# os-hxfan/BayesNN_FPGA

Measured on AMD Instinct MI355X. Metric: MCD-samples/sec (T x images/s) + ECE, ResNet-18 multi-exit T=100, higher is better.
Workload: dtype f16; 1 GPU; ResNet18MCEarlyExit C=10 dropout=block+exit p=0.25, batch 250 x T=100 (BASELINE configs[2]); batch=250, T=100, chunk_samples=102, batches_in_flight=2, hipgraph=False, macro_batches=1, pipe=2 eager batches in flight (the probed step is over 1.5 ms)

## Files before the change

### bayesnn_fpga_amd/csrc/conv3x3_s2.hip

```cpp
#include <cstdlib>

#include "conv_epilogue.h"
#include "kernels.h"

typedef _Float16 half8 __attribute__((ext_vector_type(8)));

#ifndef S2_DIRECT
#define S2_DIRECT 1
#endif
#ifndef S2_RELAX0
#define S2_RELAX0 0
#endif
#ifndef S2_DRAIN_STORES
#define S2_DRAIN_STORES 0
#endif
#ifndef S2_WSPLIT
#define S2_WSPLIT 0
#endif
#ifndef S2_STORE_SC1
#define S2_STORE_SC1 0
#endif
#ifndef S2_PIECE_PHASE
#define S2_PIECE_PHASE 1
#endif
// ... 90 lines not shown
        return (s == 0 || s == 4) ? 1 : ((s == 5 && !last) ? 1 : 0);
    }
    __host__ __device__ static constexpr int p_issued(int s, bool last) { return ((s <= 4 || !last) ? pieces_at(s) : 0) + bits_at(s, last); }
    __host__ __device__ static constexpr int wait_n(int S, bool last) {
        int n = 0;
        for (int j = S - (NST - 2); j <= S; ++j) {
            const bool prev = j < 0;
            const int sj = prev ? j + 9 : j;
            const bool lastj = last && !prev;
            if (j > S - (NST - 2)) n += w_issued(sj, lastj) ? WPI : 0;
            n += p_issued(sj, lastj);
        }
        return n;
    }
    static constexpr int WST = CT * 64;
    static constexpr int PIECE = 512 * 16;
    static constexpr int P_OFF = (NST - 1) * WST;
    static constexpr int E_OFF = P_OFF + PRO * PIECE;
    static constexpr int E_BYTES = 65536;
    static constexpr int END_PIECES = P_OFF + NPT * PIECE;
    static constexpr int WL_OFF = (END_PIECES + WST > E_OFF + E_BYTES ? END_PIECES : E_OFF + E_BYTES - WST);
    static constexpr int BN_OFF = WL_OFF + WST;
    static constexpr int BITS_OFF = BN_OFF + 2 * BN_MAX * 4 + 128;
    __host__ __device__ static constexpr int first_due(int S) {
        for (int k = 0; k < NPT; ++k)
            if (pstep(k) + 3 == S || pstep(k) + 3 == S + 9) return k;
        return -1;
    }
    static constexpr int NSLOT = MSK ? (S2_BITS_GROUP ? 3 : 6) : 0;
    __host__ __device__ static constexpr int slot(int k) { return S2_BITS_GROUP ? grp(k) : (k >= PRO ? k - PRO : (k < NA ? (k < 2 ? k : 5) : 2 + (k - NA))); }
    static_assert(!MSK || (NA == 3 && NB == 2 && NOWN == 5 && NPT == 10), "keep-bit slot plan");
    static constexpr int LUT_OFF = BITS_OFF + NSLOT * 2048;
    static constexpr int LDS_BYTES = LUT_OFF + (MSK && S2_MASK_LUT ? 4096 : 0);
    static_assert(BN_OFF - E_OFF >= E_BYTES, "epilogue staging area");
    static_assert(LDS_BYTES <= 160 * 1024, "LDS");
    __host__ __device__ static constexpr int wstage_off(int st) { return st == NST - 1 ? WL_OFF : st * WST; }
    __host__ __device__ static constexpr int p_img(int p) { return p / (TW * TW); }
    __host__ __device__ static constexpr int p_ox(int p) { return 4 * ((p >> 4) % (TW / 4)) + (p & 3); }
    __host__ __device__ static constexpr int p_oy(int p) { return 4 * (((p >> 4) / (TW / 4)) % (TW / 4)) + ((p >> 2) & 3); }
    static constexpr int BR = TW / 4, BI = BR * BR;
    __host__ __device__ static constexpr int cell_delta(int pl, int j) {
        return (j / BI) * rows(pl) * cols(pl) + 4 * ((j % BI) / BR) * cols(pl) + 4 * ((j % BI) % BR);
    }
};

__host__ __device__ constexpr int s2_plane(int s) { return s < 4 ? 0 : (s < 6 ? 1 : (s < 8 ? 2 : 3)); }
__host__ __device__ constexpr int s2_dy(int s) { return (s == 2 || s == 3 || s == 5) ? 1 : 0; }
__host__ __device__ constexpr int s2_dx(int s) { return (s == 1 || s == 3 || s == 7) ? 1 : 0; }
__host__ __device__ constexpr int s2_tap(int s) {
    constexpr int t[9] = {0, 2, 6, 8, 1, 7, 3, 5, 4};
    return t[s];
}

template <int TW, bool BF, bool IMAP, bool MSK = false, int CT_ = 256>
__global__ __launch_bounds__(512, 1) void conv3x3_s2_kernel(ConvArgs a, int n_tiles) {
    using G = S2Geom<TW, (TW == 4 ? 3 : S2_NST_BIG), MSK, CT_>;
    static_assert(!MSK || (TW == 16 && !IMAP), "masked input: one image per tile, the ordinary form");
    constexpr int CT = G::CT, IMGS = G::IMGS, NPT = G::NPT, PRO = G::PRO, NST = G::NST;
    constexpr bool HALF = CT == 128;
    constexpr int TI = 4, TP = HALF ? 4 : 8, JB = TP / 2;
    typedef float accv __attribute__((ext_vector_type(4)));
    __shared__ __attribute__((aligned(16))) char smem[G::LDS_BYTES];
    char* const pbuf = smem + G::P_OFF;
    float* const bn_scale = (float*)(smem + G::BN_OFF);
    float* const bn_bias = bn_scale + G::BN_MAX;

    const int tid = threadIdx.x;
    const int lane = tid & 63;
    const int wave = __builtin_amdgcn_readfirstlane(tid >> 6);
    const int l16 = lane & 15, kq = lane >> 4;
    const int g = wave >> 2, wc = (wave >> 1) & 1, wp = wave & 1;

    const int n_ctiles = a.Cout / CT;
    const int n_ptiles = (a.N + IMGS - 1) / IMGS;
    const int Ktot = 9 * a.Cin;
    const int nC = a.Cin / 32;
    const int split = a.wgt_b ? a.split : a.Cout;

    for (int c = tid; c < a.Cout; c += 512) {
        const bool second = c >= split;
        const float* sp = second ? a.scale_b : a.scale;
        const float* bp = second ? a.bias_b : a.bias;
        const int cc = second ? c - split : c;
        bn_scale[c] = (sp ? sp[cc] : 1.f) * a.out_mul;
        bn_bias[c] = bp ? bp[cc] : 0.f;
    }
    if constexpr (MSK && S2_MASK_LUT) {
        if (tid < 256) {
            typedef unsigned int u32x4_l __attribute__((ext_vector_type(4)));
            u32x4_l m;
#pragma unroll
            for (int i = 0; i < 4; ++i) m[i] = (((tid >> (2 * i)) & 1) ? 0xffffu : 0u) | (((tid >> (2 * i + 1)) & 1) ? 0xffff0000u : 0u);
            *(u32x4_l*)(smem + G::LUT_OFF + tid * 16) = m;
        }
    }
    __syncthreads();

    const int a_off = ((HALF ? 0 : g * 128) + wc * 64 + (S2_DIRECT ? 8 * (l16 >> 2) + (l16 & 3) : l16)) * 64 + ((kq ^ (((l16 >> 2) & 1) << 1)) << 4);
#define A_TILE(I) (S2_DIRECT ? (32 * ((I) >> 1) + 4 * ((I) & 1)) * 64 : (I) * 16 * 64)
    const int by = l16 >> 2, bx = l16 & 3;
    const int pbase = HALF ? (g * 2 + wp) * 64 : wp * 128;
    int boff[4];
#pragma unroll
    for (int pl = 0; pl < 4; ++pl) {
        const int wave_cell = G::cell0(pl) + (G::p_img(pbase) * G::rows(pl) + G::p_oy(pbase)) * G::cols(pl) + G::p_ox(pbase);
        boff[pl] = G::P_OFF + (wave_cell + by * G::cols(pl) + bx) * 64 + ((kq ^ ((by & 1) << 1)) << 4);
    }

    const unsigned HWC = (unsigned)a.H * a.W * a.Cin;
    constexpr unsigned OOB = 0xfffffff0u;
    unsigned pre[NPT];
#pragma unroll
    for (int k = 0; k < NPT; ++k) {
        const int q = tid + 512 * k;
        const int cell = q >> 2, pos = q & 3;
        const int pl = G::lo(k) == G::hi(k) ? G::lo(k) : (cell < G::cell0(G::hi(k)) ? G::lo(k) : G::hi(k));
        const int pyl = pl < 2 ? 1 : 0, pxl = (pl == 0 || pl == 2) ? 1 : 0;
        const int RQ = (TW + pyl) * (TW + pxl), Q = TW + pxl;
        const int lc = cell - (pl == 0 ? 0 : (pl == 1 ? G::cell0(1) : (pl == 2 ? G::cell0(2) : G::cell0(3))));
        const int img = lc / RQ, rm = lc - img * RQ;
        const int y = rm / Q, x = rm - y * Q;
        const int iy = 2 * y - pyl, ix = 2 * x - pxl;
        const bool ok = lc < IMGS * RQ && (unsigned)iy < (unsigned)a.H && (unsigned)ix < (unsigned)a.W;
        const unsigned inoff = (MSK && a.lazy_planar) ? (unsigned)((iy * a.W + (ix & 1) * (a.W >> 1) + (ix >> 1)) * 32 + ((pos ^ ((y & 1) << 1)) << 3))
                                                      : (unsigned)((iy * a.W + ix) * a.Cin + ((pos ^ ((y & 1) << 1)) << 3));
        pre[k] = !ok ? OOB : (IMAP ? ((unsigned)img << 24) | inoff : 2u * ((unsigned)img * HWC + inoff));
    }
    int* const row_tabs = (int*)(smem + G::BN_OFF + 2 * G::BN_MAX * 4);
    int tsel = 0;
    const unsigned woff = 2u * ((unsigned)(tid >> 2) * Ktot + (((tid & 3) ^ (((tid >> (S2_DIRECT ? 5 : 4)) & 1) << 1)) << 3));
    const unsigned wbytes = 2u * 128u * Ktot;
    const unsigned cmul = (MSK && a.lazy_planar) ? (unsigned)(a.H * a.W) : 1u;
    __amdgpu_buffer_rsrc_t rs_w0, rs_w1, rs_in, rs_bits;

    int ch0 = 0, n0 = 0;

#define BLDS16(RSRC, VOFF, SOFF, LDSPTR) \
    __builtin_amdgcn_raw_ptr_buffer_load_lds((RSRC), (__attribute__((address_space(3))) void*)(LDSPTR), 16, (VOFF), (SOFF), 0, 0)
#define ISSUE_W_HALF(KOFF, ST, I)                                                                            \
    {                                                                                                        \
        const unsigned so_ = __builtin_amdgcn_readfirstlane(2u * (unsigned)(KOFF));                          \
        if ((I) == 0) BLDS16(rs_w0, woff, so_, smem + G::wstage_off(ST) + (0 * 512 + wave * 64) * 16);       \
        else BLDS16(rs_w1, woff, so_, smem + G::wstage_off(ST) + (1 * 512 + wave * 64) * 16);                \
    }
#define ISSUE_W(KOFF, ST)                                                                                    \
    {                                                                                                        \
        ISSUE_W_HALF(KOFF, ST, 0);                                                                           \
        if (!HALF) ISSUE_W_HALF(KOFF, ST, 1);                                                                \
    }
#define ISSUE_P(K, C0)                                                                                       \
    {                                                                                                        \
        unsigned o_ = pre[K];                                                                                \
        if constexpr (IMAP) {                                                                                \
            const int row_ = row_tabs[tsel * 16 + ((pre[K] >> 24) & 15)];                                    \
            o_ = (pre[K] == OOB || row_ < 0) ? OOB : 2u * ((unsigned)row_ * HWC + (pre[K] & 0xffffffu));     \
        }                                                                                                    \
        if (!S2_ABL_NOPATCH) BLDS16(rs_in, o_, __builtin_amdgcn_readfirstlane(2u * (unsigned)(C0) * cmul), pbuf + ((K) * 512 + wave * 64) * 16); \
        if constexpr (MSK && !S2_ABL_NOBITS && !S2_BITS_GROUP) {                                             \
             \
             \
             \
            unsigned bo_ = pre[K];                                                                           \
            asm volatile("" : "+v"(bo_));                                                                    \
            __builtin_amdgcn_raw_ptr_buffer_load_lds(rs_bits, (__attribute__((address_space(3))) void*)(smem + G::BITS_OFF + G::slot(K) * 2048 + wave * 256), \
                                                     4, (bo_ >> 4) & ~3u, __builtin_amdgcn_readfirstlane(((unsigned)(C0) * cmul) >> 3), 0, 0); \
        }                                                                                                    \
    }
#define ISSUE_BITS(GRP, PA, PB, PC, PD, CB, ADD0)                                                            \
    if constexpr (MSK && !S2_ABL_NOBITS && S2_BITS_GROUP) {                                                  \
        int p4_ = tid & 3;                                                                                   \
        asm volatile("" : "+v"(p4_));                                                                        \
        unsigned bo_ = p4_ == 0 ? pre[PA] : (p4_ == 1 ? pre[PB] : ((PC) >= 0 ? (p4_ == 2 ? pre[(PC) < 0 ? 0 : (PC)] : pre[(PD) < 0 ? 0 : (PD)]) : OOB)); \
        bo_ = ((bo_ >> 4) & ~3u) + (p4_ == 0 ? (unsigned)(ADD0) : 0u);                                       \
        __builtin_amdgcn_raw_ptr_buffer_load_lds(rs_bits, (__attribute__((address_space(3))) void*)(smem + G::BITS_OFF + (GRP) * 2048 + wave * 256), \
                                                 4, bo_, __builtin_amdgcn_readfirstlane(((unsigned)(CB) * cmul) >> 3), 0, 0); \
    }
    typedef unsigned int u32x4_m __attribute__((ext_vector_type(4)));
#define MASK_LOAD(K, W, V)                                                                                   \
// ... 135 lines not shown
                    if (sn_ <= 8) { ISSUE_W_HALF(s2_tap(sn_ <= 8 ? sn_ : 0) * a.Cin + c32, st_w_, kk); }       \
                    else if (!last) { ISSUE_W_HALF(s2_tap(sn_ > 8 ? sn_ - 9 : 0) * a.Cin + c32 + 32, st_w_, kk); } \
                }                                                                                              \
            }                                                                                                  \
            if (kk == S2_PIECE_PHASE) {                                                                        \
                _Pragma("unroll") for (int k = 0; k < NPT; ++k)                                                \
                    if (G::pstep(k) == (S)) {                                                                  \
                        if (k >= PRO) { ISSUE_P(k, c32); }                                                     \
                        else if (!last) { ISSUE_P(k, c32 + 32); }                                              \
                    }                                                                                          \
                if ((S) == 0) { ISSUE_BITS(2, 5, 6, 7, 8, c32, 0); }                                           \
                if ((S) == 4) { ISSUE_BITS(1, 4, 9, -1, -1, c32, 4); }                                         \
                if ((S) == 5) { if (!last) { ISSUE_BITS(0, 0, 1, 2, 3, c32 + 32, 0); } }                       \
            }                                                                                                  \
             \
             \
            if (MSK && S2_MASK_PHASE == 2 && kk == 1) asm volatile("s_waitcnt lgkmcnt(4)" ::: "memory");       \
            if (kk == 1 && g == 1) END_OF_STEP_WAIT(S);                 \
            RAW_BARRIER();                                                                                     \
            asm volatile("s_waitcnt lgkmcnt(0)" ::: "memory");                                                 \
            __builtin_amdgcn_s_setprio(1);                                                                     \
            if constexpr (MSK && S2_MASK_PHASE == 2 && due0_ >= 0) {                                           \
                if (kk == 0) {                                                                                 \
                     \
                                        \
                    _Pragma("unroll") for (int j = 0; j < 4; ++j) acc[0][j] = mfma_16x16x32<BF>(af[0], bf[j], acc[0][j]); \
                    __builtin_amdgcn_sched_barrier(0);                                                         \
                    if (due_on_) { MASK_LOAD(due0_ < 0 ? 0 : due0_, mw0_, mv0_); }                             \
                    __builtin_amdgcn_sched_barrier(0);                                                         \
                    _Pragma("unroll") for (int i = 1; i < 3; ++i)                                              \
                        _Pragma("unroll") for (int j = 0; j < 4; ++j) acc[i][j] = mfma_16x16x32<BF>(af[i], bf[j], acc[i][j]); \
                    __builtin_amdgcn_sched_barrier(0);                                                         \
                    if (due_on_) { MASK_STORE(due0_ < 0 ? 0 : due0_, mw0_, mv0_); }                            \
                    _Pragma("unroll") for (int k = 0; k < NPT; ++k)                                            \
                        if (k != due0_ && MASK_DUE(S, k)) { if (due_on_) { MASK_P(k); } }                      \
                    __builtin_amdgcn_sched_barrier(0);                                                         \
                    _Pragma("unroll") for (int j = 0; j < 4; ++j) acc[3][j] = mfma_16x16x32<BF>(af[3], bf[j], acc[3][j]); \
                } else {                                                                                       \
                    _Pragma("unroll") for (int i = 0; i < TI; ++i)                                             \
                        _Pragma("unroll") for (int j = 0; j < JB; ++j)                                         \
                            acc[i][JB * kk + j] = mfma_16x16x32<BF>(af[i], bf[j], acc[i][JB * kk + j]);        \
                }                                                                                              \
            } else {                                                                                           \
                _Pragma("unroll") for (int i = 0; i < TI; ++i)                                                 \
                    _Pragma("unroll") for (int j = 0; j < JB; ++j)                                             \
                        acc[i][JB * kk + j] = mfma_16x16x32<BF>(af[i], bf[j], acc[i][JB * kk + j]);            \
            }                                                                                                  \
            __builtin_amdgcn_s_setprio(0);                                                                     \
            if (kk == 1 && g == 0) END_OF_STEP_WAIT(S);                 \
            RAW_BARRIER();                                                                                     \
        }                                                                                                      \
    }

    int vb = blockIdx.x, v_step = (int)gridDim.x, v_end = n_tiles;
    if (MSK && a.lazy_order) {
        if ((gridDim.x & 7) == 0) {
            const int L = (n_tiles + 7) >> 3, J = (int)gridDim.x >> 3;
            vb = (int)(blockIdx.x & 7) * L + (int)(blockIdx.x >> 3);
            v_step = J;
            v_end = (int)((blockIdx.x & 7) + 1) * L < n_tiles ? (int)((blockIdx.x & 7) + 1) * L : n_tiles;
        }
        if (vb >= v_end) return;
    }
    SETUP_TILE(vb);
    constexpr int NSTORES = HALF ? 8 : 16;
    bool stores16 = false;
    while (vb < v_end) {
        const int cur_ch0 = ch0, cur_n0 = n0, cur_tsel = tsel;
        accv acc[TI][TP];
#pragma unroll
        for (int i = 0; i < TI; ++i)
#pragma unroll
            for (int j = 0; j < TP; ++j)
#pragma unroll
                for (int e = 0; e < 4; ++e) acc[i][j][e] = 0.f;

        if (IMAP || !stores16 || S2_DRAIN_STORES) asm volatile("s_waitcnt vmcnt(0)" ::: "memory");
        else asm volatile("s_waitcnt vmcnt(%0)" ::"n"(NSTORES) : "memory");
        if constexpr (MSK) {
#pragma unroll
            for (int k = 0; k < PRO; ++k) MASK_P(k);
            asm volatile("s_waitcnt lgkmcnt(0)" ::: "memory");
        }
        RAW_BARRIER();
        if (g == 1) RAW_BARRIER();
        half8 af[TI], bf[4];
        for (int chunk = 0; chunk < nC; ++chunk) {
            const bool last = chunk + 1 == nC;
            const int c32 = chunk * 32;
            S2_STEP(0) S2_STEP(1) S2_STEP(2) S2_STEP(3) S2_STEP(4) S2_STEP(5) S2_STEP(6) S2_STEP(7) S2_STEP(8)
        }
        if (g == 0) RAW_BARRIER();
        asm volatile("s_waitcnt vmcnt(0)" ::: "memory");

        const int nvb = vb + v_step;
        if (nvb < v_end) SETUP_TILE(nvb);

        if (S2_ABL_NOEPI) {
            float sum_ = 0.f;
#pragma unroll
            for (int i = 0; i < TI; ++i)
#pragma unroll
                for (int j = 0; j < TP; ++j) sum_ += acc[i][j][0] + acc[i][j][1] + acc[i][j][2] + acc[i][j][3];
            if (sum_ == 12345.678f) a.out[tid] = (_Float16)sum_;
        } else {
            char* const E = smem + G::E_OFF + g * 32768;
            int tl = tid & 255;
            asm volatile("" : "+v"(tl));
            const int chl = cur_ch0 + (HALF ? 0 : 128 * g);
            _Float16* outp = a.out;
            int oc = a.Cout, chg = chl;
            if (a.wgt_b) {
                if (chl >= split) { outp = a.out_b; oc = a.Cout - split; chg = chl - split; }
                else oc = split;
            }
            const int k = tl & 15;
            float* const poolp = TW == 4 ? ((a.wgt_b && chl >= split) ? a.pool_b : a.pool) : nullptr;
            if (poolp) {
#pragma unroll
                for (int i = 0; i < 4; ++i) {
                    const int cw = S2_DIRECT ? 32 * (i >> 1) + 8 * kq + 4 * (i & 1) : 16 * i + 4 * kq;
                    const int c4 = chl + wc * 64 + cw;
                    const f32x4_e sc = *(const f32x4_e*)(bn_scale + c4), bi = *(const f32x4_e*)(bn_bias + c4);
#pragma unroll
                    for (int j = 0; j < TP; ++j) {
                        f32x4_e v;
#pragma unroll
                        for (int e = 0; e < 4; ++e) {
                            float x = fmaxf(__builtin_fmaf(acc[i][j][e], sc[e], bi[e]), 0.f);
                            x += __builtin_bit_cast(float, __builtin_amdgcn_update_dpp(0, __builtin_bit_cast(int, x), 0xB1, 0xF, 0xF, true));
                            x += __builtin_bit_cast(float, __builtin_amdgcn_update_dpp(0, __builtin_bit_cast(int, x), 0x4E, 0xF, 0xF, true));
                            x += __builtin_bit_cast(float, __builtin_amdgcn_update_dpp(0, __builtin_bit_cast(int, x), 0x141, 0xF, 0xF, true));
                            x += __builtin_bit_cast(float, __builtin_amdgcn_update_dpp(0, __builtin_bit_cast(int, x), 0x140, 0xF, 0xF, true));
                            v[e] = x * (1.f / 16.f);
                        }
                        int n = cur_n0 + wp * 8 + j;
                        if constexpr (IMAP) n = row_tabs[cur_tsel * 16 + wp * 8 + j];
                        else if (n >= a.N) n = -1;
                        if (l16 == 0 && n >= 0) *(f32x4_e*)(poolp + (size_t)n * oc + chg + wc * 64 + cw) = v;
                    }
                }
                if (!S2_DIRECT) { lds_barrier(); lds_barrier(); lds_barrier(); }
            } else if constexpr (S2_DIRECT) {
                const int cw = wc * 64 + 8 * kq;
                f32x4_e sc[4], bi[4];
#pragma unroll
                for (int i = 0; i < 4; ++i) {
                    sc[i] = *(const f32x4_e*)(bn_scale + chl + cw + 32 * (i >> 1) + 4 * (i & 1));
                    bi[i] = *(const f32x4_e*)(bn_bias + chl + cw + 32 * (i >> 1) + 4 * (i & 1));
                }
#pragma unroll
                for (int j = 0; j < TP; ++j) {
                    const int p = pbase + 16 * j + l16;
                    int n = cur_n0 + G::p_img(p);
                    if constexpr (IMAP) n = row_tabs[cur_tsel * 16 + G::p_img(p)];
                    else if (n >= a.N) n = -1;
                    _Float16* const dst = outp + ((size_t)(n < 0 ? 0 : n) * (TW * TW) + G::p_oy(p) * TW + G::p_ox(p)) * oc + chg + cw;
#pragma unroll
                    for (int h = 0; h < 2; ++h) {
                        half8_e o;
#pragma unroll
                        for (int ii = 0; ii < 2; ++ii)
#pragma unroll
                            for (int e = 0; e < 4; ++e) {
                                float v = acc[2 * h + ii][j][e] * sc[2 * h + ii][e] + bi[2 * h + ii][e];
                                if (a.relu) v = fmaxf(v, 0.f);
                                o[4 * ii + e] = a16_from_f32<BF>(v);
                            }
                        if (n >= 0 && !S2_ABL_NOSTORE) *(half8_e*)(dst + 32 * h) = o;
                    }
                }
            } else
#pragma unroll
            for (int rr = 0; rr < (HALF ? 1 : 2); ++rr) {
                if (rr) lds_barrier();
#pragma unroll
                for (int i = 0; i < 4; ++i) {
                    const int c4 = chl + wc * 64 + 16 * i + 4 * kq;
                    const f32x4_e sc = *(const f32x4_e*)(bn_scale + c4), bi = *(const f32x4_e*)(bn_bias + c4);
                    const int cq = wc * 8 + 2 * i + (kq >> 1);
#pragma unroll
                    for (int jj = 0; jj < 4; ++jj) {
                        const int p = wp * 64 + jj * 16 + l16;
                        half4 o;
#pragma unroll
                        for (int e = 0; e < 4; ++e) {
                            float v = acc[i][4 * rr + jj][e] * sc[e] + bi[e];
                            if (a.relu) v = fmaxf(v, 0.f);
                            o[e] = a16_from_f32<BF>(v);
                        }
                        *(half4*)(E + p * 256 + ((cq ^ l16) << 4) + (((kq ^ jj) & 1) << 3)) = o;
                    }
                }
                lds_barrier();
#pragma unroll
                for (int hb = 0; hb < 2; ++hb) {
                    half8_e o8[4];
#pragma unroll
                    for (int it = 0; it < 4; ++it) {
                        const int pl = (tl >> 4) + 16 * (4 * hb + it);
                        o8[it] = *(const half8_e*)(E + pl * 256 + ((k ^ (pl & 15)) << 4));
                    }
#pragma unroll
                    for (int it = 0; it < 4; ++it) {
                        const int pl = (tl >> 4) + 16 * (4 * hb + it);
                        const int p = HALF ? g * 128 + pl : (pl >> 6) * 128 + rr * 64 + (pl & 63);
                        int n = cur_n0 + G::p_img(p);
                        if constexpr (IMAP) n = row_tabs[cur_tsel * 16 + G::p_img(p)];
                        else if (n >= a.N) n = -1;
                        if (n < 0 || S2_ABL_NOSTORE) continue;
                        half8_e v = o8[it];
                        if (it & 1) v = __builtin_shufflevector(v, v, 4, 5, 6, 7, 0, 1, 2, 3);
                        _Float16* dst_ = outp + ((size_t)n * (TW * TW) + G::p_oy(p) * TW + G::p_ox(p)) * oc + chg + 8 * k;
                        if (S2_STORE_SC1) {
                            typedef unsigned int u32x4_ __attribute__((ext_vector_type(4)));
                            asm volatile("global_store_dwordx4 %0, %1, off sc1\n\ts_nop 1" ::"v"(dst_), "v"(__builtin_bit_cast(u32x4_, v)) : "memory");
                        } else {
                            *(half8_e*)dst_ = v;
                        }
                    }
                }
            }
        }
        stores16 = cur_n0 + IMGS <= a.N;
        vb = nvb;
    }
#undef S2_STEP
#undef END_OF_STEP_WAIT
#undef WAIT_VM
#undef RAW_BARRIER
#undef SETUP_TILE
#undef ISSUE_BITS
#undef MASK_DUE
#undef MASK_P
#undef MASK_STORE
#undef MASK_LOAD
#undef ISSUE_P
#undef ISSUE_W
#undef ISSUE_W_HALF
#undef A_TILE
}


bool conv_takes_s2_kernel(int ksize, int stride, int pad, int cin, int cout, int h, int w, int ho, int wo) {
    return ksize == 3 && stride == 2 && pad == 1 && cin % 32 == 0 && (cout % 256 == 0 || (cout % 128 == 0 && ho == 16)) &&
           cout <= (ho == 4 ? 1024 : 512) && ho == wo && (ho == 16 || ho == 8 || ho == 4) && h == 2 * ho && w == 2 * wo;
}

template <int TW>
static int launch_s2(const ConvArgs& a, int n_cu, hipStream_t s) {
    using G = S2Geom<TW>;
    const bool half = a.Cout % 256 != 0;
    const long tiles = (long)((a.N + G::IMGS - 1) / G::IMGS) * (a.Cout / (half ? 128 : 256));
    if (tiles <= 0 || tiles > 0x7fffffffL) return BMI_ERR_INVALID;
    const dim3 grid((unsigned)(tiles < n_cu ? tiles : n_cu)), block(512);
    if (half) {
        if constexpr (TW == 16) {
            if (a.wgt_b || (a.imap && a.in_bits)) return BMI_ERR_UNSUPPORTED;
            ConvArgs al = a;
            al.lazy_order = a.in_bits && opt_lazy_order() && a.in_mod < a.N && a.N % a.in_mod == 0;
            if (a.imap) {
                if (a.bf16) hipLaunchKernelGGL((conv3x3_s2_kernel<16, true, true, false, 128>), grid, block, 0, s, al, (int)tiles);
                else hipLaunchKernelGGL((conv3x3_s2_kernel<16, false, true, false, 128>), grid, block, 0, s, al, (int)tiles);
            } else if (a.in_bits) {
                if (a.bf16) hipLaunchKernelGGL((conv3x3_s2_kernel<16, true, false, true, 128>), grid, block, 0, s, al, (int)tiles);
                else hipLaunchKernelGGL((conv3x3_s2_kernel<16, false, false, true, 128>), grid, block, 0, s, al, (int)tiles);
            } else {
                if (a.bf16) hipLaunchKernelGGL((conv3x3_s2_kernel<16, true, false, false, 128>), grid, block, 0, s, al, (int)tiles);
                else hipLaunchKernelGGL((conv3x3_s2_kernel<16, false, false, false, 128>), grid, block, 0, s, al, (int)tiles);
            }
            BMI_CHECK_LAUNCH();
            return BMI_OK;
        } else {
            return BMI_ERR_UNSUPPORTED;
        }
    }
#define S2_LAUNCH(BF_, IMAP_) hipLaunchKernelGGL((conv3x3_s2_kernel<TW, BF_, IMAP_>), grid, block, 0, s, a, (int)tiles)
    if (a.in_bits) {
        if constexpr (TW == 16) {
            ConvArgs al = a;
            al.lazy_order = opt_lazy_order() && a.in_mod < a.N && a.N % a.in_mod == 0;
            if (a.bf16) hipLaunchKernelGGL((conv3x3_s2_kernel<16, true, false, true>), grid, block, 0, s, al, (int)tiles);
            else hipLaunchKernelGGL((conv3x3_s2_kernel<16, false, false, true>), grid, block, 0, s, al, (int)tiles);
        } else {
            return BMI_ERR_UNSUPPORTED;
        }
    }
    else if (a.imap) { if (a.bf16) S2_LAUNCH(true, true); else S2_LAUNCH(false, true); }
    else { if (a.bf16) S2_LAUNCH(true, false); else S2_LAUNCH(false, false); }
#undef S2_LAUNCH
    BMI_CHECK_LAUNCH();
    return BMI_OK;
}

int launch_conv3x3_s2(const ConvArgs& a_in, hipStream_t s) {
    if (!opt_conv_s2() || a_in.in2 || a_in.partial || !conv_epilogue_is_plain(a_in)) return BMI_ERR_UNSUPPORTED;
    if (a_in.in_bits && (a_in.Ho != 16 || a_in.imap || a_in.out_mul != 1.f || a_in.Cin % 32 != 0)) return BMI_ERR_UNSUPPORTED;
    if (a_in.lazy_planar && (!a_in.in_bits || (a_in.W & 1))) return BMI_ERR_UNSUPPORTED;
    if (!conv_takes_s2_kernel(a_in.ksize, a_in.stride, a_in.pad, a_in.Cin, a_in.Cout, a_in.H, a_in.W, a_in.Ho, a_in.Wo)) return BMI_ERR_UNSUPPORTED;
    ConvArgs a = a_in;
    if (a.N <= 0 || a.in_mod <= 0 || a.B <= 0) return BMI_ERR_INVALID;
    if (a.wgt_b && (!a.out_b || a.split <= 0 || a.split >= a.Cout || a.split % 128 != 0)) return BMI_ERR_INVALID;
    if ((a.pool || a.pool_b) && a.Ho != 4) return BMI_ERR_UNSUPPORTED;
    if (a.imap && (size_t)a.in_mod * a.H * a.W * a.Cin >= 0x7fffffffull) return BMI_ERR_UNSUPPORTED;
    if (a.in_mod < a.N && !a.imap && a.Ho != 16) return BMI_ERR_UNSUPPORTED;
    if ((size_t)a.H * a.W * a.Cin >= (1u << 24)) return BMI_ERR_UNSUPPORTED;
    static const int n_cu = [] {
        int dev = 0, cu = 0;
        if (hipGetDevice(&dev) != hipSuccess || hipDeviceGetAttribute(&cu, hipDeviceAttributeMultiprocessorCount, dev) != hipSuccess) cu = 0;
        return cu > 0 ? cu : 256;
    }();
    if (opt_conv_s2() != 2) {
        const int imgs = 256 / (a.Ho * a.Wo), n_sel = a.n_ref > 0 ? a.n_ref : a.N;
        if ((long)((n_sel + imgs - 1) / imgs) * (a.Cout / (a.Cout % 256 ? 128 : 256)) < 3 * n_cu / 4) return BMI_ERR_UNSUPPORTED;
    }
    a.xcd_split = xcd_split_for(a.Cout / (a.Cout % 256 ? 128 : 256), (size_t)a.Cout * 9 * a.Cin * 2);
    return a.Ho == 16 ? launch_s2<16>(a, n_cu, s) : (a.Ho == 8 ? launch_s2<8>(a, n_cu, s) : launch_s2<4>(a, n_cu, s));
}
```

### bayesnn_fpga_amd/csrc/engine.hip

```cpp
#include <algorithm>
#include <cmath>
#include <cstdlib>
#include <cstring>
#include <new>
#include <vector>

#include "conv_epilogue.h"
#include "kernels.h"

namespace {

struct TensorInfo {
    int h = 0, w = 0, c = 0;
    bool stoch = false;
    bool bits = false;
    bool f32 = false;
    bool dense_out = false;
    bool pooled_now = false;
    int lazy_bits = -1, lazy_scaled = -1;
    bool lazy_planar_plan = false;
    bool lazy_planar = false;
    bool lazy_pending = false;
    bool lazy_planar_now = false;
    EltArgs lazy_call;
// ... 110 lines not shown
    {
        *family = BMI_CONV_FAMILY_S2;
        const int rc = launch_conv3x3_s2(a, s);
        if (rc != BMI_ERR_UNSUPPORTED) return rc;
    }
    if (opt_conv_wide()) {
        *family = BMI_CONV_FAMILY_WIDE;
        const int rc = launch_conv_igemm_wide(a, s);
        if (rc != BMI_ERR_UNSUPPORTED) return rc;
    }
    *family = BMI_CONV_FAMILY_IGEMM;
    return launch_conv_igemm(a, s);
}

static bool site_ok(const bmi_site& s) {
    switch (s.kind) {
        case BMI_SITE_NONE: return true;
        case BMI_SITE_ELEMENTWISE:
        case BMI_SITE_CHANNEL: return s.p >= 0.f && s.p <= 1.f && s.site_id >= 0;
        case BMI_SITE_MASKSEMBLE: return s.num_masks > 0 && s.masks != nullptr && s.site_id >= 0;
        default: return false;
    }
}

static int shape_from_env(const char* primary, const char* fallback) {
    const char* v = std::getenv(primary);
    if (!v && fallback) v = std::getenv(fallback);
    const int x = v ? std::atoi(v) : 0;
    return x == 16 || x == 32 ? x : BMI_DEFAULT_MFMA_SHAPE;
}
static BmiOptions initial_options() {
    BmiOptions o;
    o.mfma_shape_patch = shape_from_env("BMI_MFMA_SHAPE", nullptr);
    o.mfma_shape_wide = shape_from_env("BMI_MFMA_SHAPE_WIDE", "BMI_MFMA_SHAPE");
    o.unit_dtype = BMI_DTYPE_F16;
    const char* e = std::getenv("BMI_XCD_SPLIT");
    const int x = e ? std::atoi(e) : 0;
    o.xcd_split = x == 1 || x == 2 || x == 4 ? x : 0;
    return o;
}
BmiOptions& bmi_default_options() { static BmiOptions o = initial_options(); return o; }
thread_local const BmiOptions* bmi_tl_options = nullptr;
static int unit_pair() { const int d = opt_unit_dtype(); return d == BMI_DTYPE_F16X2 ? 1 : (d == BMI_DTYPE_BF16X3 ? 2 : 0); }
static bool unit_f32act() { const int d = opt_unit_dtype(); return d == BMI_DTYPE_F32 || d == BMI_DTYPE_F16X2 || d == BMI_DTYPE_BF16X3; }

static int set_named_option(BmiOptions& o, const char* name, int32_t value) {
    if (!name) return BMI_ERR_INVALID;
    struct Row { const char* name; int BmiOptions::*field; int lo, hi; };
    static const Row rows[] = {
        {"unit_entry_dtype", &BmiOptions::unit_dtype, BMI_DTYPE_F16, BMI_DTYPE_BF16X3},
        {"pw_persist", &BmiOptions::pw_persist, 0, 1},
        {"pw_pad_skip", &BmiOptions::pw_pad_skip, 0, 1},
        {"pw_pad_skip8", &BmiOptions::pw_pad_skip8, 0, 1},
        {"lazy_planar", &BmiOptions::lazy_planar, 0, 1},
        {"ws_no_reuse", &BmiOptions::ws_no_reuse, 0, 1},
        {"wide_persist_min_x10", &BmiOptions::wide_persist_min, 10, 1000},
        {"conv_pw", &BmiOptions::conv_pw, 0, 4},
        {"conv_s2", &BmiOptions::conv_s2, 0, 2},
        {"conv_pool", &BmiOptions::conv_pool, 0, 2},
        {"mask_lazy", &BmiOptions::mask_lazy, 0, 1},
        {"conv_wide", &BmiOptions::conv_wide, 0, 1},
        {"split_shx", &BmiOptions::split_shx, 0, 2},
        {"split_tile", &BmiOptions::split_tile, 0, 1},
        {"conv_seam", &BmiOptions::conv_seam, 0, 3},
        {"conv_stream", &BmiOptions::conv_stream, 0, 3},
        {"splitk", &BmiOptions::splitk, 0, 1},
        {"dense_exact", &BmiOptions::dense_exact, 0, 1},
        {"lazy_order", &BmiOptions::lazy_order, 0, 1},
        {"epilogue_lite", &BmiOptions::epilogue_lite, 0, 2},
        {"head_batch", &BmiOptions::head_batch, 0, 1},
        {"conv_patch64", &BmiOptions::conv_patch64, 0, 1},
        {"splitk_tiles", &BmiOptions::splitk_tiles, 0, 1024},
        {"pair_prefix", &BmiOptions::pair_prefix, 0, 1},
        {"patch_direct", &BmiOptions::patch_direct, 0, 2},
    };
    for (const Row& r : rows)
        if (std::strcmp(name, r.name) == 0) {
            if (value < r.lo || value > r.hi) return BMI_ERR_INVALID;
            o.*(r.field) = value;
            return BMI_OK;
        }
    if (std::strcmp(name, "xcd_split") == 0) {
        if (value != 0 && value != 1 && value != 2 && value != 4) return BMI_ERR_INVALID;
        o.xcd_split = value;
        return BMI_OK;
    }
    const bool patch = std::strcmp(name, "mfma_shape_patch") == 0, wide = std::strcmp(name, "mfma_shape_wide") == 0;
    if (!patch && !wide) return BMI_ERR_INVALID;
    if (value != 0 && value != 16 && value != 32) return BMI_ERR_INVALID;
    (patch ? o.mfma_shape_patch : o.mfma_shape_wide) = value ? value : BMI_DEFAULT_MFMA_SHAPE;
    return BMI_OK;
}
int xcd_split_for(int n_ctiles, size_t weight_bytes) {
    int cs = opt_xcd_split();
    if (cs == 0) cs = weight_bytes > (8u << 20) ? 4 : (weight_bytes > (3u << 20) ? 2 : 1);
    while (cs > 1 && n_ctiles % cs != 0) cs >>= 1;
    return cs;
}

int op_stage(const OpInfo& op, int first_exit) { return std::max(0, op.xstage - first_exit); }

bool prefix_row_form(const bmi_engine_s* h, const OpInfo& op) {
    const bmi_op_desc& d = op.d;
    if (d.kind == BMI_OP_STEM) return false;
    if (d.kind != BMI_OP_CONV || h->f32 || d.ksize != 1 || op.has_pair || op.nsplit > 1 || d.in2 >= 0) return true;
    const TensorInfo& tin = h->tensors[d.in];
// ... 1756 lines not shown
```

### bayesnn_fpga_amd/csrc/kernels.h

```cpp
#pragma once
#include <hip/hip_runtime.h>
#include <stdint.h>

#include "../../include/bayesnn_fpga_amd.h"
#include "philox.h"

struct ConvArgs {
    const _Float16* in;
    const _Float16* wgt;
    const float* scale;
    const float* bias;
    const _Float16* res;
    const uint8_t* res_bits;
    const uint8_t* in_bits;
    float out_mul;
    const _Float16* in2;
    const _Float16* wgt2;
    int in2_mod, H2, W2, Cin2, stride2;
    const _Float16* wgt_b;
    const float* scale_b;
    const float* bias_b;
    _Float16* out_b;
    int split;
    float* pool;
// ... 97 lines not shown
                              const double* SH, double* mean, double* var, double* lm, double* pred, double* expd, double* mi, int* nonfinite,
                              hipStream_t s);
int launch_mask_permute(const float* src, float* dst, int m, int c, int cnt0, int stride, hipStream_t s);
int launch_exit_rule_decide(const double* S1, int B, int C, int t_total, double thr, int margin, int ensemble, const int* in, int bc, int* out,
                            int* count, int* exit_of, int e, hipStream_t s);
int launch_expand_rows(const int* active, int bc, int batch, int tc, int* rows, hipStream_t s);
int launch_finalize(int64_t n, int t_total, const double* S1, const double* S2, const double* SL, double* mean,
                    double* var, double* lm, int* nonfinite, hipStream_t s);
int launch_finalize_uncertainty(int n_rows, int C, int t_total, const double* S1, const double* SH, double* pred, double* expd,
                                double* mi, int* nonfinite, hipStream_t s);
int launch_nll_temperature_grid(const float* logits, int T, int E, int B, int C, const int* labels, const float* tau_grid, int G, double* nll,
                                double* scratch, hipStream_t s);
#define BMI_ENS_MAX_EXITS 32
#define BMI_ENS_MAX_CLASSES 128
bool ensemble_takes(int E, int C);
int launch_ensemble_moments(const float* logits, int T, int E, int B, int C, const float* inv_tau, double* Q1, double* Q2, double* QH,
                            hipStream_t s, const int* list = nullptr, int Bc = 0, const int* n_e = nullptr);
int launch_exit_counts(const int* exit_of, int n, int* n_e, hipStream_t s);
int launch_finalize_ensemble(int n_rows, int C, int t_total, const double* Q1, const double* Q2, const double* QH, double* mean, double* var,
                             double* pred, double* expd, double* mi, int* nonfinite, hipStream_t s);
int launch_finalize_ensemble_per_image(int n_exits, int batch, int C, const int* t_used, const double* Q1, const double* Q2, const double* QH,
                                       double* mean, double* var, double* pred, double* expd, double* mi, int* nonfinite, hipStream_t s);
int launch_philox_mask(uint8_t* keep, int64_t n, uint64_t seed, int site, int t, float p, hipStream_t s);
int launch_mask_bits(uint8_t* bits, int n, int hw, int c, const SiteArgs& site, int batch, int t0, hipStream_t s, int planar_w = 0);
int launch_scale_copy(const _Float16* in, _Float16* out, long n, float scale, int bf16, hipStream_t s, int planar_hw = 0, int planar_w = 0, int planar_c = 0);
int launch_splitk_finish(const ConvArgs& a, hipStream_t s);
int launch_conv1x1_seam(const ConvArgs& a, const ConvArgs& b, hipStream_t s);
bool conv_takes_seam_kernel(int cmid, int cw, int cn);
bool conv1x1_stream_takes(const ConvArgs& a);
int launch_conv1x1_stream(const ConvArgs& a, hipStream_t s);
bool conv_takes_patch_kernel(int ksize, int stride, int pad, int cin, int cout, int ho, int wo);

struct BmiOptions {
    int mfma_shape_patch = 0, mfma_shape_wide = 0;
    int unit_dtype = 0;
    int wide_persist_min = 10;
    int conv_pw = 1;
    int conv_wide = 1;
    int mask_lazy = 1;
    int conv_pool = 1;
    int conv_s2 = 1;
    int split_shx = 1;
    int split_tile = 1;
    int conv_seam = 1;
    int conv_stream = 1;
    int splitk = 1;
    int dense_exact = 0;
    int lazy_order = 1;
    int epilogue_lite = 1;
    int xcd_split = 0;
    int pw_persist = 1;
    int pw_pad_skip = 1;
    int pw_pad_skip8 = 1;
    int lazy_planar = 1;
    int ws_no_reuse = 0;
    int conv_patch64 = 1;
    int splitk_tiles = 64;
    int pair_prefix = 1;
    int patch_direct = 1;
    int head_batch = 1;
};
BmiOptions& bmi_default_options();
extern thread_local const BmiOptions* bmi_tl_options;
inline const BmiOptions& bmi_options() { return bmi_tl_options ? *bmi_tl_options : bmi_default_options(); }
struct BmiOptionScope {
    const BmiOptions* prev;
    explicit BmiOptionScope(const BmiOptions* o) : prev(bmi_tl_options) { bmi_tl_options = o; }
    ~BmiOptionScope() { bmi_tl_options = prev; }
    BmiOptionScope(const BmiOptionScope&) = delete;
    BmiOptionScope& operator=(const BmiOptionScope&) = delete;
};
#define BMI_OPT(name) inline int opt_##name() { return bmi_options().name; }
BMI_OPT(mfma_shape_patch) BMI_OPT(mfma_shape_wide) BMI_OPT(unit_dtype) BMI_OPT(wide_persist_min) BMI_OPT(conv_pw) BMI_OPT(conv_wide)
BMI_OPT(mask_lazy) BMI_OPT(conv_pool) BMI_OPT(conv_s2) BMI_OPT(split_shx) BMI_OPT(split_tile) BMI_OPT(conv_seam) BMI_OPT(conv_stream)
BMI_OPT(splitk) BMI_OPT(dense_exact) BMI_OPT(lazy_order) BMI_OPT(epilogue_lite) BMI_OPT(xcd_split) BMI_OPT(pw_persist) BMI_OPT(lazy_planar)
BMI_OPT(pw_pad_skip) BMI_OPT(pw_pad_skip8) BMI_OPT(ws_no_reuse) BMI_OPT(head_batch) BMI_OPT(conv_patch64) BMI_OPT(splitk_tiles) BMI_OPT(pair_prefix) BMI_OPT(patch_direct)
#undef BMI_OPT
int xcd_split_for(int n_ctiles, size_t weight_bytes);

SiteArgs resolve_site(const bmi_site* site, uint64_t seed, int mask_cnt0, uint64_t elem_off = 0);

#define BMI_CHECK_LAUNCH()                                  \
    do {                                                    \
        hipError_t e__ = hipGetLastError();                 \
        if (e__ != hipSuccess) return BMI_ERR_HIP;          \
    } while (0)
```

Baseline: 1.243 million MCD-samples/s.

## Skip MFMAs on padding taps in stride-2 8x8->4x4 conv with new pool epilogue

Adds a specialized stride-2 conv kernel for the 4x4-output class that remaps pixel-to-lane assignment so each wave's tiles follow image-per-lane order, letting it statically skip MFMAs and B-fragment loads for (position, tap) pairs that read only zero padding (121 of 144 live). It also adds a pooled-output epilogue that reduces across the paired pixel waves through LDS, plus adjusted store waits. The cost is a new code path with more barriers, doubled unrolled code per wave parity and imbalance between the two pixel waves (61 of 72 steps on the slower one). It is enabled by default.

```diff
diff --git a/bayesnn_fpga_amd/csrc/conv3x3_s2.hip b/bayesnn_fpga_amd/csrc/conv3x3_s2.hip
--- a/bayesnn_fpga_amd/csrc/conv3x3_s2.hip
+++ b/bayesnn_fpga_amd/csrc/conv3x3_s2.hip
@@ -166,10 +166,46 @@
     return t[s];
 }
 
-template <int TW, bool BF, bool IMAP, bool MSK = false, int CT_ = 256>
-__global__ __launch_bounds__(512, 1) void conv3x3_s2_kernel(ConvArgs a, int n_tiles) {
+struct S2Skip {
+    __host__ __device__ static constexpr int t_y(int j) { return j >> 1; }
+    __host__ __device__ static constexpr int t_x(int wp, int j) { return 2 * (j & 1) + (((j >> 1) + wp) & 1); }
+    __host__ __device__ static constexpr bool valid(int wp, int j, int S) {
+        return !((s2_tap(S) / 3 == 0 && t_y(j) == 0) || (s2_tap(S) % 3 == 0 && t_x(wp, j) == 0));
+    }
+    __host__ __device__ static constexpr int cell(int wp, int j, int S) {
+        return (t_y(j) + s2_dy(S)) * (4 + ((s2_plane(S) & 1) ? 0 : 1)) + t_x(wp, j) + s2_dx(S);
+    }
+    __host__ __device__ static constexpr int count(int wp, int S) { int n = 0; for (int t = 0; t < 8; ++t) n += valid(wp, t, S) ? 1 : 0; return n; }
+    __host__ __device__ static constexpr int phase(int wp, int j, int S) {
+        int r = 0;
+        for (int t = 0; t < j; ++t) r += valid(wp, t, S) ? 1 : 0;
+        return r < (count(wp, S) + 1) / 2 ? 0 : 1;
+    }
+    __host__ __device__ static constexpr bool live(int wp, int j, int S, int kk) { return valid(wp, j, S) && phase(wp, j, S) == kk; }
+    __host__ __device__ static constexpr unsigned mask(int wp, int S, int kk) { unsigned m = 0; for (int j = 0; j < 8; ++j) m |= live(wp, j, S, kk) ? 1u << j : 0u; return m; }
+    __host__ __device__ static constexpr int sum(int wp) { int n = 0; for (int s = 0; s < 9; ++s) n += count(wp, s); return n; }
+    __host__ __device__ static constexpr int slower() { int n = 0; for (int s = 0; s < 9; ++s) n += count(0, s) > count(1, s) ? count(0, s) : count(1, s); return n; }
+    __host__ __device__ static constexpr bool cells_ok() {
+        for (int wp = 0; wp < 2; ++wp)
+            for (int j = 0; j < 8; ++j)
+                for (int s = 0; s < 9; ++s) {
+                    const int pl = s2_plane(s), y = t_y(j) + s2_dy(s), x = t_x(wp, j) + s2_dx(s);
+                    const bool pad = (pl < 2 && y == 0) || ((pl == 0 || pl == 2) && x == 0);
+                    if (valid(wp, j, s) == pad) return false;
+                    if (y >= S2Geom<4>::rows(pl) || x >= S2Geom<4>::cols(pl) || cell(wp, j, s) != y * S2Geom<4>::cols(pl) + x) return false;
+                }
+        return true;
+    }
+};
+static_assert(S2Skip::slower() == 61 && S2Skip::sum(0) + S2Skip::sum(1) == 121, "pad-skip: 61 of 72 tile-steps per chunk on the slower pixel wave, 121 of 144 live (position, tap) pairs");
+static_assert(S2Skip::count(0, 0) == 5 && S2Skip::count(1, 0) == 4 && S2Skip::count(0, 8) == 8 && S2Skip::count(1, 4) == 6, "pad-skip: live tiles per tap");
+static_assert(S2Skip::cells_ok(), "pad-skip: a tile is dead exactly when it reads the padding row / column of its plane");
+
+template <int TW, bool BF, bool IMAP, bool MSK, int CT_, bool SKIP>
+__device__ __forceinline__ void conv3x3_s2_body(const ConvArgs& a, int n_tiles) {
     using G = S2Geom<TW, (TW == 4 ? 3 : S2_NST_BIG), MSK, CT_>;
     static_assert(!MSK || (TW == 16 && !IMAP), "masked input: one image per tile, the ordinary form");
+    static_assert(!SKIP || (TW == 4 && CT_ == 256 && !IMAP && !MSK && S2_DIRECT && !S2_WSPLIT && !S2_RELAX0), "pad-skip: the 8x8 -> 4x4 class without a row table");
     constexpr int CT = G::CT, IMGS = G::IMGS, NPT = G::NPT, PRO = G::PRO, NST = G::NST;
     constexpr bool HALF = CT == 128;
     constexpr int TI = 4, TP = HALF ? 4 : 8, JB = TP / 2;
@@ -219,6 +255,7 @@
     for (int pl = 0; pl < 4; ++pl) {
         const int wave_cell = G::cell0(pl) + (G::p_img(pbase) * G::rows(pl) + G::p_oy(pbase)) * G::cols(pl) + G::p_ox(pbase);
         boff[pl] = G::P_OFF + (wave_cell + by * G::cols(pl) + bx) * 64 + ((kq ^ ((by & 1) << 1)) << 4);
+        if constexpr (SKIP) boff[pl] = G::P_OFF + (G::cell0(pl) + l16) * 64 + ((kq ^ (((l16 >> 3) & 1) << 1)) << 4);
     }
 
     const unsigned HWC = (unsigned)a.H * a.W * a.Cin;
@@ -232,12 +269,13 @@
         const int pyl = pl < 2 ? 1 : 0, pxl = (pl == 0 || pl == 2) ? 1 : 0;
         const int RQ = (TW + pyl) * (TW + pxl), Q = TW + pxl;
         const int lc = cell - (pl == 0 ? 0 : (pl == 1 ? G::cell0(1) : (pl == 2 ? G::cell0(2) : G::cell0(3))));
-        const int img = lc / RQ, rm = lc - img * RQ;
+        const int img = SKIP ? (lc & 15) : lc / RQ, rm = SKIP ? (lc >> 4) : lc - img * RQ;
         const int y = rm / Q, x = rm - y * Q;
         const int iy = 2 * y - pyl, ix = 2 * x - pxl;
+        const int sw = SKIP ? ((img >> 3) & 1) : (y & 1);
         const bool ok = lc < IMGS * RQ && (unsigned)iy < (unsigned)a.H && (unsigned)ix < (unsigned)a.W;
-        const unsigned inoff = (MSK && a.lazy_planar) ? (unsigned)((iy * a.W + (ix & 1) * (a.W >> 1) + (ix >> 1)) * 32 + ((pos ^ ((y & 1) << 1)) << 3))
-                                                      : (unsigned)((iy * a.W + ix) * a.Cin + ((pos ^ ((y & 1) << 1)) << 3));
+        const unsigned inoff = (MSK && a.lazy_planar) ? (unsigned)((iy * a.W + (ix & 1) * (a.W >> 1) + (ix >> 1)) * 32 + ((pos ^ (sw << 1)) << 3))
+                                                      : (unsigned)((iy * a.W + ix) * a.Cin + ((pos ^ (sw << 1)) << 3));
         pre[k] = !ok ? OOB : (IMAP ? ((unsigned)img << 24) | inoff : 2u * ((unsigned)img * HWC + inoff));
     }
     int* const row_tabs = (int*)(smem + G::BN_OFF + 2 * G::BN_MAX * 4);
@@ -479,6 +517,52 @@
         }                                                                                                      \
     }
 
+#define S2_STEP_S(S, WP)                                                                                       \
+    {                                                                                                          \
+        constexpr int pl_ = s2_plane(S), sn_ = (S) + NST - 1;                                                  \
+        constexpr int st_r_ = (S) % 3, st_w_ = ((S) + 2) % 3;                                                  \
+        constexpr unsigned live_[2] = {S2Skip::mask(WP, S, 0), S2Skip::mask(WP, S, 1)};                        \
+        constexpr int cols_ = G::cols(pl_), shift_ = s2_dy(S) * cols_ + s2_dx(S);        \
+        static_assert(S2Skip::cell(WP, 5, S) == (5 >> 1) * cols_ + 2 * (5 & 1) + (((5 >> 1) + (WP)) & 1) + shift_, "cell"); \
+        const char* ws_ = smem + G::wstage_off(st_r_) + a_off;                                                 \
+        const char* pb_ = smem + boff[pl_];                                                                    \
+        _Pragma("unroll") for (int kk = 0; kk < 2; ++kk) {                                                     \
+            if (kk == 0) {                                                                                     \
+                _Pragma("unroll") for (int i = 0; i < TI; ++i) af[i] = *(const half8*)(ws_ + A_TILE(i));       \
+            }                                                                                                  \
+            _Pragma("unroll") for (int j = 0; j < TP; ++j)                                                     \
+                if ((live_[kk] >> j) & 1u) bfs[j] = *(const half8*)(pb_ + ((j >> 1) * cols_ + 2 * (j & 1) + (((j >> 1) + (WP)) & 1) + shift_) * 1024); \
+            if (kk == 0) {                                                                                     \
+                if (sn_ <= 8) { ISSUE_W(s2_tap(sn_ <= 8 ? sn_ : 0) * a.Cin + c32, st_w_); }                    \
+                else if (!last) { ISSUE_W(s2_tap(sn_ > 8 ? sn_ - 9 : 0) * a.Cin + c32 + 32, st_w_); }          \
+            }                                                                                                  \
+            if (kk == S2_PIECE_PHASE) {                                                                        \
+                _Pragma("unroll") for (int k = 0; k < NPT; ++k)                                                \
+                    if (G::pstep(k) == (S)) {                                                                  \
+                        if (k >= PRO) { ISSUE_P(k, c32); }                                                     \
+                        else if (!last) { ISSUE_P(k, c32 + 32); }                                              \
+                    }                                                                                          \
+            }                                                                                                  \
+            if (kk == 1 && g == 1) END_OF_STEP_WAIT(S);                                                        \
+            RAW_BARRIER();                                                                                     \
+            asm volatile("s_waitcnt lgkmcnt(0)" ::: "memory");                                                 \
+            __builtin_amdgcn_s_setprio(1);                                                                     \
+            _Pragma("unroll") for (int i = 0; i < TI; ++i)                                                     \
+                _Pragma("unroll") for (int j = 0; j < TP; ++j)                                                 \
+                    if ((live_[kk] >> j) & 1u) acc[i][j] = mfma_16x16x32<BF>(af[i], bfs[j], acc[i][j]);        \
+            __builtin_amdgcn_s_setprio(0);                                                                     \
+            if (kk == 1 && g == 0) END_OF_STEP_WAIT(S);                                                        \
+            RAW_BARRIER();                                                                                     \
+        }                                                                                                      \
+    }
+#define S2_CHUNKS_S(WP)                                                                                        \
+    for (int chunk = 0; chunk < nC; ++chunk) {                                                                 \
+        const bool last = chunk + 1 == nC;                                                                     \
+        const int c32 = chunk * 32;                                                                            \
+        S2_STEP_S(0, WP) S2_STEP_S(1, WP) S2_STEP_S(2, WP) S2_STEP_S(3, WP) S2_STEP_S(4, WP)                   \
+        S2_STEP_S(5, WP) S2_STEP_S(6, WP) S2_STEP_S(7, WP) S2_STEP_S(8, WP)                                    \
+    }
+
     int vb = blockIdx.x, v_step = (int)gridDim.x, v_end = n_tiles;
     if (MSK && a.lazy_order) {
         if ((gridDim.x & 7) == 0) {
@@ -492,6 +576,7 @@
     SETUP_TILE(vb);
     constexpr int NSTORES = HALF ? 8 : 16;
     bool stores16 = false;
+    [[maybe_unused]] bool pooled_prev = false;
     while (vb < v_end) {
         const int cur_ch0 = ch0, cur_n0 = n0, cur_tsel = tsel;
         accv acc[TI][TP];
@@ -503,6 +588,10 @@
                 for (int e = 0; e < 4; ++e) acc[i][j][e] = 0.f;
 
         if (IMAP || !stores16 || S2_DRAIN_STORES) asm volatile("s_waitcnt vmcnt(0)" ::: "memory");
+        else if (SKIP && pooled_prev) {
+            if (wp) asm volatile("s_waitcnt vmcnt(0)" ::: "memory");
+            else asm volatile("s_waitcnt vmcnt(4)" ::: "memory");
+        }
         else asm volatile("s_waitcnt vmcnt(%0)" ::"n"(NSTORES) : "memory");
         if constexpr (MSK) {
 #pragma unroll
@@ -511,11 +600,17 @@
         }
         RAW_BARRIER();
         if (g == 1) RAW_BARRIER();
-        half8 af[TI], bf[4];
-        for (int chunk = 0; chunk < nC; ++chunk) {
-            const bool last = chunk + 1 == nC;
-            const int c32 = chunk * 32;
-            S2_STEP(0) S2_STEP(1) S2_STEP(2) S2_STEP(3) S2_STEP(4) S2_STEP(5) S2_STEP(6) S2_STEP(7) S2_STEP(8)
+        half8 af[TI];
+        if constexpr (SKIP) {
+            half8 bfs[TP];
+            if (wp == 0) { S2_CHUNKS_S(0) } else { S2_CHUNKS_S(1) }
+        } else {
+            half8 bf[4];
+            for (int chunk = 0; chunk < nC; ++chunk) {
+                const bool last = chunk + 1 == nC;
+                const int c32 = chunk * 32;
+                S2_STEP(0) S2_STEP(1) S2_STEP(2) S2_STEP(3) S2_STEP(4) S2_STEP(5) S2_STEP(6) S2_STEP(7) S2_STEP(8)
+            }
         }
         if (g == 0) RAW_BARRIER();
         asm volatile("s_waitcnt vmcnt(0)" ::: "memory");
@@ -523,6 +618,7 @@
         const int nvb = vb + v_step;
         if (nvb < v_end) SETUP_TILE(nvb);
 
+        [[maybe_unused]] bool pooled_now = false;
         if (S2_ABL_NOEPI) {
             float sum_ = 0.f;
 #pragma unroll
@@ -543,7 +639,80 @@
             }
             const int k = tl & 15;
             float* const poolp = TW == 4 ? ((a.wgt_b && chl >= split) ? a.pool_b : a.pool) : nullptr;
-            if (poolp) {
+            if constexpr (SKIP) pooled_now = poolp != nullptr;
+            if (SKIP && poolp) {
+                if constexpr (SKIP) {
+                char* const X = smem + G::E_OFF;
+                char* const mine_x = X + wave * 8192 + lane * 16;
+                char* const theirs_x = X + (wave ^ 1) * 8192 + lane * 16;
+                const int chw = chl + wc * 64 + 8 * kq;
+#pragma unroll
+                for (int h = 0; h < 2; ++h) {
+                    f32x4_e sc[2], bi[2];
+#pragma unroll
+                    for (int ii = 0; ii < 2; ++ii) {
+                        sc[ii] = *(const f32x4_e*)(bn_scale + chw + 32 * h + 4 * ii);
+                        bi[ii] = *(const f32x4_e*)(bn_bias + chw + 32 * h + 4 * ii);
+                    }
+                    float xs[TP][8];
+#pragma unroll
+                    for (int j = 0; j < TP; ++j)
+#pragma unroll
+                        for (int ii = 0; ii < 2; ++ii)
+#pragma unroll
+                            for (int e = 0; e < 4; ++e) xs[j][4 * ii + e] = fmaxf(__builtin_fmaf(acc[2 * h + ii][j][e], sc[ii][e], bi[ii][e]), 0.f);
+#pragma unroll
+                    for (int jj = 0; jj < 4; ++jj)
+#pragma unroll
+                        for (int q = 0; q < 2; ++q) {
+                            f32x4_e t;
+#pragma unroll
+                            for (int e = 0; e < 4; ++e) t[e] = wp ? xs[jj][4 * q + e] : xs[4 + jj][4 * q + e];
+                            *(f32x4_e*)(mine_x + (jj * 2 + q) * 1024) = t;
+                        }
+                    lds_barrier();
+                    float rs[2][8];
+#pragma unroll
+                    for (int r = 0; r < 2; ++r)
+#pragma unroll
+                        for (int q = 0; q < 2; ++q) {
+                            const f32x4_e t0 = *(const f32x4_e*)(theirs_x + ((2 * r) * 2 + q) * 1024), t1 = *(const f32x4_e*)(theirs_x + ((2 * r + 1) * 2 + q) * 1024);
+#pragma unroll
+                            for (int e = 0; e < 4; ++e) {
+                                const float o0 = wp ? xs[4 + 2 * r][4 * q + e] : xs[2 * r][4 * q + e], o1 = wp ? xs[4 + 2 * r + 1][4 * q + e] : xs[2 * r + 1][4 * q + e];
+                                const float s01 = o0 + t0[e], s23 = o1 + t1[e];
+                                rs[r][4 * q + e] = s01 + s23;
+                            }
+                        }
+                    float half_sum[8];
+#pragma unroll
+                    for (int c = 0; c < 8; ++c) half_sum[c] = rs[0][c] + rs[1][c];
+                    lds_barrier();
+                    if (wp) {
+#pragma unroll
+                        for (int q = 0; q < 2; ++q) {
+                            f32x4_e t;
+#pragma unroll
+                            for (int e = 0; e < 4; ++e) t[e] = half_sum[4 * q + e];
+                            *(f32x4_e*)(theirs_x + q * 1024) = t;
+                        }
+                    }
+                    lds_barrier();
+                    if (!wp) {
+                        const int n = cur_n0 + l16;
+#pragma unroll
+                        for (int q = 0; q < 2; ++q) {
+                            const f32x4_e t = *(const f32x4_e*)(mine_x + q * 1024);
+                            f32x4_e pv;
+#pragma unroll
+                            for (int e = 0; e < 4; ++e) pv[e] = (half_sum[4 * q + e] + t[e]) * (1.f / 16.f);
+                            if (n < a.N) *(f32x4_e*)(poolp + (size_t)n * oc + chg + wc * 64 + 8 * kq + 32 * h + 4 * q) = pv;
+                        }
+                    }
+                }
+                asm volatile("s_waitcnt lgkmcnt(0)" ::: "memory");
+                }
+            } else if (poolp) {
 #pragma unroll
                 for (int i = 0; i < 4; ++i) {
                     const int cw = S2_DIRECT ? 32 * (i >> 1) + 8 * kq + 4 * (i & 1) : 16 * i + 4 * kq;
@@ -579,10 +748,11 @@
 #pragma unroll
                 for (int j = 0; j < TP; ++j) {
                     const int p = pbase + 16 * j + l16;
-                    int n = cur_n0 + G::p_img(p);
+                    int n = cur_n0 + (SKIP ? l16 : G::p_img(p));
+                    const int opos = SKIP ? S2Skip::t_y(j) * TW + S2Skip::t_x(wp, j) : G::p_oy(p) * TW + G::p_ox(p);
                     if constexpr (IMAP) n = row_tabs[cur_tsel * 16 + G::p_img(p)];
                     else if (n >= a.N) n = -1;
-                    _Float16* const dst = outp + ((size_t)(n < 0 ? 0 : n) * (TW * TW) + G::p_oy(p) * TW + G::p_ox(p)) * oc + chg + cw;
+                    _Float16* const dst = outp + ((size_t)(n < 0 ? 0 : n) * (TW * TW) + opos) * oc + chg + cw;
 #pragma unroll
                     for (int h = 0; h < 2; ++h) {
                         half8_e o;
@@ -595,6 +765,13 @@
                                 o[4 * ii + e] = a16_from_f32<BF>(v);
                             }
                         if (n >= 0 && !S2_ABL_NOSTORE) *(half8_e*)(dst + 32 * h) = o;
+                    }
+                }
+                if constexpr (SKIP) {
+                    const float* const pool_o = (a.wgt_b && cur_ch0 + 128 * (1 - g) >= split) ? a.pool_b : a.pool;
+                    if (pool_o) {
+#pragma unroll
+                        for (int b = 0; b < 6; ++b) lds_barrier();
                     }
                 }
             } else
@@ -649,9 +826,12 @@
                 }
             }
         }
+        if constexpr (SKIP) pooled_prev = pooled_now;
         stores16 = cur_n0 + IMGS <= a.N;
         vb = nvb;
     }
+#undef S2_CHUNKS_S
+#undef S2_STEP_S
 #undef S2_STEP
 #undef END_OF_STEP_WAIT
 #undef WAIT_VM
@@ -666,6 +846,16 @@
 #undef ISSUE_W
 #undef ISSUE_W_HALF
 #undef A_TILE
+}
+
+template <int TW, bool BF, bool IMAP, bool MSK = false, int CT_ = 256>
+__global__ __launch_bounds__(512, 1) void conv3x3_s2_kernel(ConvArgs a, int n_tiles) {
+    conv3x3_s2_body<TW, BF, IMAP, MSK, CT_, false>(a, n_tiles);
+}
+
+template <bool BF>
+__global__ __launch_bounds__(512, 1) void conv3x3_s2_skip_kernel(ConvArgs a, int n_tiles) {
+    conv3x3_s2_body<4, BF, false, false, 256, true>(a, n_tiles);
 }
 
 
@@ -703,6 +893,14 @@
         }
     }
 #define S2_LAUNCH(BF_, IMAP_) hipLaunchKernelGGL((conv3x3_s2_kernel<TW, BF_, IMAP_>), grid, block, 0, s, a, (int)tiles)
+    if constexpr (TW == 4) {
+        if (opt_s2_pad_skip() && !a.imap && !a.in_bits) {
+            if (a.bf16) hipLaunchKernelGGL((conv3x3_s2_skip_kernel<true>), grid, block, 0, s, a, (int)tiles);
+            else hipLaunchKernelGGL((conv3x3_s2_skip_kernel<false>), grid, block, 0, s, a, (int)tiles);
+            BMI_CHECK_LAUNCH();
+            return BMI_OK;
+        }
+    }
     if (a.in_bits) {
         if constexpr (TW == 16) {
             ConvArgs al = a;
diff --git a/bayesnn_fpga_amd/csrc/engine.hip b/bayesnn_fpga_amd/csrc/engine.hip
--- a/bayesnn_fpga_amd/csrc/engine.hip
+++ b/bayesnn_fpga_amd/csrc/engine.hip
@@ -186,6 +186,7 @@
         {"pw_persist", &BmiOptions::pw_persist, 0, 1},
         {"pw_pad_skip", &BmiOptions::pw_pad_skip, 0, 1},
         {"pw_pad_skip8", &BmiOptions::pw_pad_skip8, 0, 1},
+        {"s2_pad_skip", &BmiOptions::s2_pad_skip, 0, 1},
         {"lazy_planar", &BmiOptions::lazy_planar, 0, 1},
         {"ws_no_reuse", &BmiOptions::ws_no_reuse, 0, 1},
         {"wide_persist_min_x10", &BmiOptions::wide_persist_min, 10, 1000},
diff --git a/bayesnn_fpga_amd/csrc/kernels.h b/bayesnn_fpga_amd/csrc/kernels.h
--- a/bayesnn_fpga_amd/csrc/kernels.h
+++ b/bayesnn_fpga_amd/csrc/kernels.h
@@ -173,6 +173,7 @@
     int pw_persist = 1;
     int pw_pad_skip = 1;
     int pw_pad_skip8 = 1;
+    int s2_pad_skip = 1;
     int lazy_planar = 1;
     int ws_no_reuse = 0;
     int conv_patch64 = 1;
@@ -195,7 +196,7 @@
 BMI_OPT(mfma_shape_patch) BMI_OPT(mfma_shape_wide) BMI_OPT(unit_dtype) BMI_OPT(wide_persist_min) BMI_OPT(conv_pw) BMI_OPT(conv_wide)
 BMI_OPT(mask_lazy) BMI_OPT(conv_pool) BMI_OPT(conv_s2) BMI_OPT(split_shx) BMI_OPT(split_tile) BMI_OPT(conv_seam) BMI_OPT(conv_stream)
 BMI_OPT(splitk) BMI_OPT(dense_exact) BMI_OPT(lazy_order) BMI_OPT(epilogue_lite) BMI_OPT(xcd_split) BMI_OPT(pw_persist) BMI_OPT(lazy_planar)
-BMI_OPT(pw_pad_skip) BMI_OPT(pw_pad_skip8) BMI_OPT(ws_no_reuse) BMI_OPT(head_batch) BMI_OPT(conv_patch64) BMI_OPT(splitk_tiles) BMI_OPT(pair_prefix) BMI_OPT(patch_direct)
+BMI_OPT(pw_pad_skip) BMI_OPT(pw_pad_skip8) BMI_OPT(s2_pad_skip) BMI_OPT(ws_no_reuse) BMI_OPT(head_batch) BMI_OPT(conv_patch64) BMI_OPT(splitk_tiles) BMI_OPT(pair_prefix) BMI_OPT(patch_direct)
 #undef BMI_OPT
 int xcd_split_for(int n_ctiles, size_t weight_bytes);
 
```

Measured after the change: 1.262 million MCD-samples/s (median of 6 runs). +1.6%, better.
